# anzeA/Tarok

Measured on AMD Instinct MI355X. Metric: env steps/sec at 65 536 parallel 4-player games; 1/2/4/8 MI355X, higher is better.
Workload: dtype u64

## Files before the change

### tarok_amd/csrc/tarok_env.hip

```cpp
#include "tarok_device.h"

#include <hip/hip_runtime.h>
#include <stdint.h>
#include <stdio.h>
#include <stdlib.h>
#include <string.h>
#include <type_traits>
#include <utility>

#include "../../include/tarok_env.h"

#define TK_BLOCK 256
#define TK_PF_SLOTS (4 * TK_BLOCK)
#define TK_GRAPH_CACHE 16
#define TK_REFILL_CAP (TK_BLOCK * TK_AHEAD)
#define TK_REFILL_FAN 8
#define TK_RC(group, k) ((((size_t)(group)) * 4 + (k)) * 32)
#define TK_BULK_EVERY 32u
#define TK_BULK_CAP ((TK_BULK_EVERY / 4) * TK_BLOCK)

#define TK_AHEAD TAROK_GAMES_AHEAD
#define TK_LINE(episode) ((u32)(episode) % (u32)TK_AHEAD)
#define TK_FINQ 128
#define TK_STREAM_STORE(ptr, val) __builtin_nontemporal_store((val), (ptr))
#define TK_WAIT_LOADS() __builtin_amdgcn_s_waitcnt(0x0F70)
#define TK_RARE(c) __builtin_expect(!!(c), 0)
#define TK_USUAL(c) __builtin_expect(!!(c), 1)

struct __attribute__((aligned(64))) AuxLine {
    ulonglong2 n01, n23; u64 nkey; u32 nep;
    u32 pad[5];
};
struct __attribute__((aligned(64))) Aux { AuxLine line[TK_AHEAD]; };
static_assert(sizeof(AuxLine) == 64 && sizeof(Aux) == 64 * TK_AHEAD, "64 bytes per next-game line");
static_assert((TK_BLOCK * sizeof(Aux)) % 128 == 0, "a play group's next-game lines end on an L2 line boundary");
static_assert(TK_AHEAD >= 2 && TK_AHEAD <= 15, "epar / cprev are 4-bit fields");
struct __attribute__((aligned(32))) Counters {
    int4 score_sum;
    u32 episode;
    u32 pad[3];
};
static_assert(sizeof(Counters) == 32, "Counters is half a cache line");

struct tarok_env {
    int device;
    int64_t n;
    u64 offset, seed;
    int mix, flags;
    ulonglong2 *s01, *s23;
    Aux *aux;
    Counters *cnt;
    uint16_t *nstale;
    u64 *gkey;
    uint8_t *hist;
    u64 *rlist;
    u32 *rcount;
    u64 *elist;
    u32 *epoch;
    uint32_t refill_fan;
    uint32_t lazy_refill;
    int n_cus;
    float *adam_sumsq;
    u64 *stamps;
    size_t stamps_words;
    int launched;
    hipStream_t cap_stream;
    struct GraphEntry {
        hipGraphExec_t exec;
        int fused, chunk, flags, prefetch;
        void *action, *reward, *done, *obs, *stamps;
        uint32_t fan, lazy;
    } graphs[TK_GRAPH_CACHE];
    int n_graphs;
};

static thread_local int g_last_hip = 0;

#define HIPCHK(x)                                                   \
    do {                                                            \
        hipError_t e_ = (x);                                        \
        if (e_ != hipSuccess) { g_last_hip = (int)e_; return TAROK_EHIP; } \
    } while (0)

static inline dim3 grid_for(int64_t n) { return dim3((unsigned)((n + TK_BLOCK - 1) / TK_BLOCK)); }

// ... 270 lines not shown
            u32 base = 0;
#pragma unroll
            for (u32 r = 0; r < TK_REFILL_FAN; r++) base = (r == q) ? cum[r] : base;
            u64 en = tk_ld(&lists[((int64_t)(g0 + q) * 2 + which) * cap + (j - base)]);
            deal_into_buffer(aux, (int64_t)(g0 + q) * TK_BLOCK + (u32)(en & 0xFFFF), (u32)(en >> 32), seed, offset, mix);
        }
    }
    if (any || bulk) {
        __syncthreads();
        if (any && tid < fan && g0 + tid < play_groups) rcount[TK_RC(g0 + tid, par ^ 1u)] = 0u;
        if (bulk && tid < fan && g0 + tid < play_groups) rcount[TK_RC(g0 + tid, 2 + which)] = 0u;
    }
}

template <bool HIST>
__device__ __forceinline__ void play_role(
    u32 group, u32 tid,
    int64_t n, u64 seed, u64 offset, int mix, int flags, int cards, int64_t stride, TkCount count, u32 *epoch, u32 play_groups, u32 fan,
    uint8_t *__restrict__ action_out, int16_t *__restrict__ reward,
    uint8_t *__restrict__ done, uint16_t *__restrict__ trick, u64 *__restrict__ obs, uint8_t *__restrict__ hist,
    ulonglong2 *__restrict__ s01, ulonglong2 *__restrict__ s23, Aux *aux, Counters *__restrict__ cnt,
    u64 *__restrict__ gkey, u64 *rlist, u32 *rcount, u64 *__restrict__ stamps) {
    __shared__ unsigned short push_list[TK_REFILL_CAP];
    __shared__ u32 push_ep[TK_BLOCK];
    __shared__ u32 push_count;
    __shared__ u32 finq[TK_BLOCK / 64][9][TK_FINQ];
    __shared__ int sacc[4][TK_BLOCK];
    if (tid == 0) push_count = 0;
    sacc[0][tid] = 0; sacc[1][tid] = 0; sacc[2][tid] = 0; sacc[3][tid] = 0;
    __syncthreads();
    u32 fq_head = 0, fq_n = 0;
    u32 (*fq)[TK_FINQ] = finq[tid >> 6];
    auto drain_finished = [&](u32 cnt_) __attribute__((always_inline)) {
        u32 lane = tid & 63;
        if (lane < cnt_) {
            u32 e = (fq_head + lane) & (TK_FINQ - 1);
            Game f;
            f.A = TK_U64(fq[0][e], fq[1][e]); f.B = TK_U64(fq[2][e], fq[3][e]); f.C = TK_U64(fq[4][e], fq[5][e] & 0x3FFFFFu);
            u32 m = fq[7][e], ri = fq[8][e];
            f.talon = TK_U64(fq[6][e], (m >> 24) & 15u);
            f.contract = m & 15; f.declarer = (m >> 4) & 3; f.king = (m >> 6) & 3; f.team = (m >> 8) & 15;
            f.tl = (m >> 12) & 7; f.trick_no = (m >> 16) & 15; f.leader = (m >> 20) & 3;
            f.trick = 0; f.nt = 0; f.phase = TK_PHASE_DONE; f.error = 0; f.epar = 0; f.cprev = 0;
            u64 sc = final_scores(f);
            u32 t = ri & 0xFFFFu;
            if (reward) {
                u64 rs = sc;
                if ((flags & TAROK_REWARD_REF) && (f.contract == TK_BERAC || f.contract == TK_ODPRTI_BERAC)) {
                    int dv = f.trick_no >= 12 ? -20 : 20;
                    u32 d = f.declarer;
                    rs = pack_scores(d == 0 ? (int)(int16_t)(sc & 0xFFFF) : dv, d == 1 ? (int)(int16_t)((sc >> 16) & 0xFFFF) : dv,
                                     d == 2 ? (int)(int16_t)((sc >> 32) & 0xFFFF) : dv, d == 3 ? (int)(int16_t)(sc >> 48) : dv);
                }
                reinterpret_cast<u64 *>(reward)[(int64_t)group * TK_BLOCK + t + (int64_t)(ri >> 16) * stride] = rs;
            }
            atomicAdd(&sacc[0][t], (int)(int16_t)(sc & 0xFFFF)); atomicAdd(&sacc[1][t], (int)(int16_t)((sc >> 16) & 0xFFFF));
            atomicAdd(&sacc[2][t], (int)(int16_t)((sc >> 32) & 0xFFFF)); atomicAdd(&sacc[3][t], (int)(int16_t)(sc >> 48));
        }
        fq_head = (fq_head + cnt_) & (TK_FINQ - 1);
        fq_n -= cnt_;
    };
    u64 t_real0 = 0, t_cyc0 = 0, t_play = 0;
    if (stamps) { t_real0 = __builtin_amdgcn_s_memrealtime(); t_cyc0 = __builtin_amdgcn_s_memtime(); }
    int64_t i = (int64_t)group * TK_BLOCK + tid;
    bool valid = i < n;
    int64_t ic = valid ? i : n - 1;
    Game g;
    load_game(g, s01, s23, ic);
    u64 key = gkey[ic];
    bool autoreset = (flags & TAROK_AUTO_RESET) != 0;
    bool berac = g.contract == TK_BERAC || g.contract == TK_ODPRTI_BERAC;
    bool spec = valid && ((g.phase == TK_PHASE_PLAY && (int)g.nt + cards >= 4 &&
                           (berac || (int)(g.trick_no * 4 + g.nt) + cards >= 48)) ||
                          g.phase == TK_PHASE_DONE);
    u32 cprev0 = valid ? g.cprev : 0u;
    u32 allowed = TK_AHEAD - min(cprev0, (u32)TK_AHEAD);
    int4 acc = make_int4(0, 0, 0, 0);
    u32 cur_ep = 0;
    ulonglong2 na = make_ulonglong2(0, 0), nb = na, na2 = na, nb2 = na;
    u64 nkey = 0, nkey2 = 0;
    u32 nep1 = 0, nep2 = 0;
    bool ok1 = false, ok2 = false;
    auto line_tag = [&](bool &ok, u32 &nep, u32 tag) __attribute__((always_inline)) { nep = tag; ok = true; };
    if (spec) {
        acc = cnt[i].score_sum;
        cur_ep = cnt[i].episode;
        if (autoreset && allowed > 0) {
            const AuxLine *ln = &aux[i].line[TK_LINE(g.epar + 1)];
            na = ln->n01; nb = ln->n23; nkey = ln->nkey;
            line_tag(ok1, nep1, ln->nep);
            if (allowed > 1 && cards > 4) {
                const AuxLine *l2 = &aux[i].line[TK_LINE(g.epar + 2)];
                na2 = l2->n01; nb2 = l2->n23; nkey2 = l2->nkey;
                line_tag(ok2, nep2, l2->nep);
            }
        }
    }
    TK_WAIT_LOADS();
    u32 par = launch_phase<1>(count, play_groups, fan) & 1u;
    launch_counted<1>(epoch);
    g.cprev = 0;
    u32 consumed = 0;
    bool resync = false;
    bool blocked = false;
    bool acc_dirty = false, seats_dirty = false, touched = false;
    u64 legal = (valid && g.phase == TK_PHASE_PLAY) ? legal_now(g) : 0;
    u64 c_lead = 0;
    u32 legal_hi = 0;
    u64 pending = 0;
    u32 blocked_v = 0, resync_v = 0;
    auto fetch_lines = [&](bool lacks, bool lacks2) __attribute__((always_inline)) {
        if (lacks) {
            const AuxLine *ln = &aux[i].line[TK_LINE(cur_ep + 1)];
            na = ln->n01; nb = ln->n23; nkey = ln->nkey;
            line_tag(ok1, nep1, ln->nep);
        }
        if (lacks2) {
            const AuxLine *l2 = &aux[i].line[TK_LINE(cur_ep + 2)];
            na2 = l2->n01; nb2 = l2->n23; nkey2 = l2->nkey;
            line_tag(ok2, nep2, l2->nep);
        }
    };
    auto play_card = [&](auto all_tag, auto nt_tag, auto std_tag, int64_t row, int ci) __attribute__((always_inline)) {
        constexpr bool ALL = decltype(all_tag)::value;
        constexpr int NT = decltype(nt_tag)::value;
        constexpr bool STD = decltype(std_tag)::value;
        if constexpr (NT >= 0) g.nt = (u32)NT;
        constexpr bool TOP_UP_EARLY = ALL && NT == 0;
        constexpr bool TOP_UP_LATE = !(ALL && NT == 3);
        if constexpr (TOP_UP_EARLY) {
            if (TK_RARE(pending != 0)) {
                pending = 0;
                bool base = spec && blocked_v == 0 && consumed >= 1;
                bool lacks = base && nep1 != cur_ep + 1 && consumed < allowed;
                bool lacks2 = base && nep2 != cur_ep + 2 && consumed + 1 < allowed;
                fetch_lines(lacks, lacks2);
            }
        }
        const bool v = ALL ? true : valid;
        const bool play = ALL ? true : (valid && g.phase == TK_PHASE_PLAY);
        constexpr bool ALIGNED = ALL && NT >= 0;
        u32 a;
        if constexpr (ALL && NT >= 1) a = policy_action_follow(key, g.trick_no * 4 + g.nt, TK_LO(legal) | TK_HI(legal), legal_hi);
        else a = play ? policy_action(key, g.trick_no * 4 + g.nt, legal) : 255u;
        u64 scores = 0;
        u32 trick_info = 0;
        int res = -2;
        const u32 pos = g.trick_no * 4 + g.nt;
        if constexpr (ALL && NT == 0) c_lead = g.C;
        const u64 *lead_plane = (ALL && NT >= 0) ? &c_lead : nullptr;
        if (play) res = apply_step<true, true>(g, a, scores, trick_info, !STD && trick != nullptr, lead_plane);
        bool fin = res == 1;
        if (HIST && hist && play && res >= 0) hist[(int64_t)pos * n + i] = (uint8_t)a;
        if constexpr (!(ALL && NT >= 0)) {
            touched = touched || res != -2;
            seats_dirty = seats_dirty || (res >= 0 && g.nt == 0);
        }
        if (v) {
            if (STD || action_out) TK_STREAM_STORE(&action_out[row], (uint8_t)a);
            if (!STD && trick) TK_STREAM_STORE(&trick[row], (uint16_t)trick_info);
        }
        constexpr bool CAN_END = !(ALL && NT >= 0 && NT < 3);
        constexpr bool FAST_RENEW = ALL && NT == 3;
        auto push_finished = [&](u64 fm, u32 slot0) __attribute__((always_inline)) {
            u32 e = (slot0 + __builtin_amdgcn_mbcnt_hi((u32)(fm >> 32), __builtin_amdgcn_mbcnt_lo((u32)fm, 0))) & (TK_FINQ - 1);
            fq[0][e] = TK_LO(g.A); fq[1][e] = TK_HI(g.A); fq[2][e] = TK_LO(g.B); fq[3][e] = TK_HI(g.B);
            fq[4][e] = TK_LO(g.C); fq[5][e] = TK_HI(g.C); fq[6][e] = TK_LO(g.talon);
            u32 m = (g.declarer << 4) | g.contract;      TK_KEEP_VGPR(m);
            m = (g.king << 6) | m;                       TK_KEEP_VGPR(m);
            m = (g.team << 8) | m;                       TK_KEEP_VGPR(m);
            m = (g.tl << 12) | m;                        TK_KEEP_VGPR(m);
            m = (g.trick_no << 16) | m;                  TK_KEEP_VGPR(m);
            m = (g.leader << 20) | m;                    TK_KEEP_VGPR(m);
            fq[7][e] = (TK_HI(g.talon) << 24) | m;
            fq[8][e] = ((u32)ci << 16) | tid;
        };
        auto swap_in = [&]() __attribute__((always_inline)) {
            unpack_fresh(g, na.x, na.y, nb.x, nb.y);
            if constexpr (ALIGNED) g.C |= TK_C_PAD;
            key = nkey;
            na = na2; nb = nb2; nkey = nkey2;
            nep1 = nep2;
        };
        auto deal_in_place = [&](bool deal_here, Game &gd, u64 &kd) __attribute__((always_inline)) {
            u64 pend = __ballot(deal_here);
            if (TK_RARE(pend != 0)) {
                u64 dkey = 0;
                if (deal_here) dkey = game_key(seed, offset + (u64)i, cur_ep + 1);
                u64 h0 = 0, h1 = 0, h2 = 0, h3 = 0, tal = 0;
                u32 lane = __lane_id();
                while (pend) {
                    int l = __builtin_ctzll(pend);
                    pend &= pend - 1;
                    u32 klo = (u32)__builtin_amdgcn_readlane((int)(u32)dkey, l);
                    u32 khi = (u32)__builtin_amdgcn_readlane((int)(u32)(dkey >> 32), l);
                    u64 w0, w1, w2, w3, wt;
                    deal_wave(klo, khi, w0, w1, w2, w3, wt);
                    if (lane == (u32)l) { h0 = w0; h1 = w1; h2 = w2; h3 = w3; tal = wt; }
                }
                if (deal_here) {
                    u32 cc, d, k;
                    sample_setup(dkey, mix, cc, d, k);
                    setup_game(gd, h0, h1, h2, h3, tal, cc, d, k);
                    gd.epar = TK_LINE(cur_ep + 1); gd.cprev = 0;
                    if (gd.phase == TK_PHASE_EXCHANGE) bot_exchange(gd, dkey);
                    kd = dkey;
                }
            }
        };
        if constexpr (FAST_RENEW) {
            u64 fm = __ballot(fin);
            if (TK_USUAL(fm != 0)) {
                if (TK_RARE(fq_n >= 64)) drain_finished(64);
                const u32 slot0 = fq_head + fq_n;
                fq_n += (u32)__popcll(fm);
                if (TK_RARE((fm & __ballot(nep1 != cur_ep + 1)) != 0)) {
                    bool lineless = fin && nep1 != cur_ep + 1;
                    resync_v |= (lineless && consumed < allowed) ? 1u : 0u;
                    blocked_v |= lineless ? 1u : 0u;
                    Game d = g;
                    u64 dk = key;
                    deal_in_place(lineless, d, dk);
                    if (lineless) { pack(d, na.x, na.y, nb.x, nb.y); nkey = dk; nep1 = cur_ep + 1; }
                }
                pending |= fm & __ballot(nep2 != cur_ep + 2);
                if (fin) { push_finished(fm, slot0); swap_in(); cur_ep++; consumed++; }
            }
        }
        if constexpr (CAN_END && !FAST_RENEW) {
            u64 fm = __ballot(fin);
            if (TK_USUAL(fm != 0)) {
                if (TK_RARE(fq_n >= 64)) drain_finished(64);
                if (fin) push_finished(fm, fq_head + fq_n);
                fq_n += (u32)__popcll(fm);
            }
        }
        if (CAN_END && !FAST_RENEW && (ALL || autoreset)) {
            bool renew = ALL ? fin : (v && g.phase == TK_PHASE_DONE);
            if (TK_USUAL(__ballot(renew) != 0)) {
                if constexpr (TOP_UP_LATE) {
                    bool lacks = spec && !blocked && !ok1 && consumed >= 1 && consumed < allowed;
                    if (TK_RARE(__ballot(renew && lacks) != 0)) {
                        bool lacks2 = spec && !blocked && !ok2 && consumed >= 1 && consumed + 1 < allowed;
                        fetch_lines(lacks, lacks2);
                        TK_WAIT_LOADS();
                    }
                }
                bool swap = renew && !blocked && ok1 && nep1 == cur_ep + 1;
                if (swap) {
                    swap_in();
                    ok1 = ok2 && consumed + 1 < allowed;
                    ok2 = false;
                }
                bool deal_here = renew && !swap;
                if (deal_here && consumed < allowed) resync = true;
                if (deal_here) blocked = true;
                deal_in_place(deal_here, g, key);
                if (renew) { cur_ep++; consumed++; seats_dirty = true; }
            }
        }
        if constexpr (ALIGNED && NT < 3) legal = legal_mask_follow(hand_of<true>(g, (g.leader + g.nt) & 3), g.trick & 63, g.contract, legal_hi);
        else if constexpr (ALIGNED) legal = legal_mask(hand_of<true>(g, g.leader), false, 0u, g.contract);
        else legal = (ALL || (v && g.phase == TK_PHASE_PLAY)) ? legal_now(g) : 0;
        if (v) {
            const u32 fin01 = ALL ? (u32)res : (fin ? 1u : 0u);
            TK_STREAM_STORE(&obs[row], obs_word_with<true>(g, false, legal) | ((u64)(ALL ? fin01 : ((fin || g.phase == TK_PHASE_DONE) ? 1u : 0u)) << 62));
            if (STD || done) TK_STREAM_STORE(&done[row], (uint8_t)fin01);
        }
    };
    int64_t row = i;
    typedef std::integral_constant<int, -1> nt_any;
    if (autoreset && __ballot(valid && g.phase == TK_PHASE_PLAY) == ~0ULL) {
        if ((cards & 3) == 0 && __ballot(g.nt != 0) == 0) {
            auto tricks = [&](auto std_tag) __attribute__((always_inline)) {
                touched = true; seats_dirty = true;
                g.C |= TK_C_PAD;
                for (int c = 0; c < cards; c += 4) {
                    play_card(std::true_type{}, std::integral_constant<int, 0>{}, std_tag, row, c); row += stride;
                    play_card(std::true_type{}, std::integral_constant<int, 1>{}, std_tag, row, c + 1); row += stride;
                    play_card(std::true_type{}, std::integral_constant<int, 2>{}, std_tag, row, c + 2); row += stride;
                    play_card(std::true_type{}, std::integral_constant<int, 3>{}, std_tag, row, c + 3); row += stride;
                }
                g.C &= TK_DECK;
            };
            if (action_out && done && !trick) tricks(std::true_type{});
            else tricks(std::false_type{});
        } else {
            for (int c = 0; c < cards; c++, row += stride) play_card(std::true_type{}, nt_any{}, std::false_type{}, row, c);
        }
    } else {
        for (int c = 0; c < cards; c++, row += stride) play_card(std::false_type{}, nt_any{}, std::false_type{}, row, c);
    }
    while (fq_n) drain_finished(min(fq_n, 64u));
    __builtin_amdgcn_s_waitcnt(0xC07F);
    {
        int4 sa = make_int4(sacc[0][tid], sacc[1][tid], sacc[2][tid], sacc[3][tid]);
        if (sa.x | sa.y | sa.z | sa.w) { acc.x += sa.x; acc.y += sa.y; acc.z += sa.z; acc.w += sa.w; acc_dirty = true; }
    }
    u32 np = (resync || resync_v != 0) ? (u32)TK_AHEAD : min(consumed, (u32)TK_AHEAD);
    if (valid) {
        g.cprev = np;
        if (acc_dirty) cnt[i].score_sum = acc;
        if (consumed) { cnt[i].episode = cur_ep; gkey[i] = key; }
        if (touched || consumed || cprev0 != np) store_game(g, s01, s23, i, seats_dirty || cprev0 != np);
    }
    if (stamps) t_play = __builtin_amdgcn_s_memtime() - t_cyc0;
    if (valid && np) {
        u32 pos = atomicAdd(&push_count, np);
        push_ep[tid] = cur_ep;
        for (u32 j = 0; j < np; j++) push_list[pos + j] = (unsigned short)(j * TK_BLOCK + tid);
    }
    __syncthreads();
    u32 total = push_count;
    u64 *lst = rlist + ((int64_t)group * 2 + par) * TK_REFILL_CAP;
    for (u32 j = tid; j < total; j += TK_BLOCK) {
        u32 en = push_list[j], t = en % TK_BLOCK;
        lst[j] = ((u64)(push_ep[t] + TK_AHEAD - en / TK_BLOCK) << 32) | t;
    }
    if (tid == 0) rcount[TK_RC(group, par)] = total;
    if (stamps && (tid & 63) == 0) {
        u64 w = (u64)i >> 6;
        stamps[3 * w + 0] = t_real0;
        stamps[3 * w + 1] = __builtin_amdgcn_s_memrealtime();
        stamps[3 * w + 2] = ((__builtin_amdgcn_s_memtime() - t_cyc0) << 32) | (t_play & 0xFFFFFFFFULL);
    }
}

#define TK_PLAY_ARGS                                                                                                             \
    int64_t n, u64 seed, u64 offset, int mix, int flags, int cards, int64_t stride, u32 play_groups, u32 *epoch, u32 fan,         \
        uint8_t *__restrict__ action_out, int16_t *__restrict__ reward,                                                           \
        uint8_t *__restrict__ done, uint16_t *__restrict__ trick, u64 *__restrict__ obs, uint8_t *__restrict__ hist,              \
        ulonglong2 *__restrict__ s01, ulonglong2 *__restrict__ s23, Aux *aux, Counters *__restrict__ cnt,                         \
        u64 *__restrict__ gkey, u64 *rlist, u32 *rcount, u64 *__restrict__ stamps
template <bool HIST>
TK_KERNEL(TK_BLOCK, 168) __attribute__((amdgpu_waves_per_eu(3, 3))) void k_play_wide(TK_PLAY_ARGS) {
    TK_VGPR_TOP(168, 167);
    TkCount count = launch_count<1>(epoch, play_groups);
    if (blockIdx.x >= play_groups)
        refill_role<false>(blockIdx.x - play_groups, threadIdx.x, TK_BLOCK, seed, offset, mix, play_groups, count, epoch, fan, false, aux, rlist, rcount, nullptr);
    else {
        play_role<HIST>(blockIdx.x, threadIdx.x, n, seed, offset, mix, flags, cards, stride, count, epoch, play_groups, fan,
                        action_out, reward, done, trick, obs, hist, s01, s23, aux, cnt, gkey, rlist, rcount, stamps);
    }
}

__device__ __forceinline__ void deal_in_place_wave(bool deal_here, Game &gd, u64 &kd, u64 seed, u64 offset, int64_t i, u32 ep, int mix) {
    u64 pend = __ballot(deal_here);
    if (pend == 0) return;
    u64 dkey = 0;
    if (deal_here) dkey = game_key(seed, offset + (u64)i, ep);
    u64 h0 = 0, h1 = 0, h2 = 0, h3 = 0, tal = 0;
    u32 lane = __lane_id();
    while (pend) {
        int l = __builtin_ctzll(pend);
        pend &= pend - 1;
        u32 klo = (u32)__builtin_amdgcn_readlane((int)(u32)dkey, l);
// ... 1123 lines not shown
    TK_VGPR_TOP(64, 63);
    int64_t i = (int64_t)blockIdx.x * TK_BLOCK + threadIdx.x;
    if (i >= n) return;
    if (ep) ep[i] = cnt[i].episode;
    if (score_sum) score_sum[i] = cnt[i].score_sum;
}

TK_KERNEL(TK_BLOCK, 64) void k_get_state(int64_t n, const ulonglong2 *__restrict__ s01,
                                                       const ulonglong2 *__restrict__ s23, u64 *__restrict__ out) {
    TK_VGPR_TOP(64, 63);
    int64_t i = (int64_t)blockIdx.x * TK_BLOCK + threadIdx.x;
    if (i >= n) return;
    Game g;
    load_game(g, s01, s23, i);
    u64 on_table = 0;
    for (u32 j = 0; j < g.nt; j++) on_table |= 1ULL << ((g.trick >> (6 * j)) & 63);
    u64 won = g.C & ~talon_unowned(g) & ~on_table;
    for (u32 s = 0; s < 4; s++) {
        out[(int64_t)s * n + i] = hand_of(g, s);
        out[(int64_t)(4 + s) * n + i] = seat_cards(g, s) & won;
    }
    out[8 * n + i] = g.talon;
    u64 m = g.trick;
    m |= (u64)g.nt << 24;
    m |= (u64)g.leader << 27;
    m |= (u64)g.trick_no << 29;
    m |= (u64)g.contract << 33;
    m |= (u64)g.declarer << 37;
    m |= (u64)(has_king(g.contract) ? g.king : 7) << 39;
    m |= (u64)g.team << 42;
    m |= (u64)(g.contract == TK_KLOP ? g.tl : 0) << 46;
    m |= (u64)(has_exchange(g.contract) ? g.tl : 7) << 49;
    m |= (u64)g.phase << 52;
    m |= (u64)g.error << 54;
    out[9 * n + i] = m;
}

TK_KERNEL(TK_BLOCK, 64) void k_set_state(int64_t n, const u64 *__restrict__ in,
                                                       ulonglong2 *__restrict__ s01, ulonglong2 *__restrict__ s23,
                                                       const Counters *__restrict__ cnt) {
    TK_VGPR_TOP(64, 63);
    int64_t i = (int64_t)blockIdx.x * TK_BLOCK + threadIdx.x;
    if (i >= n) return;
    u64 m = in[9 * n + i];
    Game g;
    g.trick = (u32)m & 0xFFFFFF;
    g.nt = (u32)(m >> 24) & 7; g.leader = (u32)(m >> 27) & 3; g.trick_no = (u32)(m >> 29) & 15;
    g.contract = (u32)(m >> 33) & 15; g.declarer = (u32)(m >> 37) & 3;
    u32 king = (u32)(m >> 39) & 7;
    g.king = king == 7 ? 0 : king;
    g.team = (u32)(m >> 42) & 15;
    u32 talon_left = (u32)(m >> 46) & 7, choice = (u32)(m >> 49) & 7;
    g.phase = (u32)(m >> 52) & 3; g.error = (u32)(m >> 54) & 1;
    g.epar = TK_LINE(cnt[i].episode);
    {
        ulonglong2 old = s23[i];
        g.cprev = ((u32)(old.y >> 62) & 3u) | (((u32)(old.x >> 62) & 3u) << 2);
    }
    g.talon = in[8 * n + i] & ((1ULL << 36) - 1);
    g.tl = g.contract == TK_KLOP ? talon_left : ((has_exchange(g.contract) || g.contract == TK_SOLO_BREZ) ? choice : 0);
    u64 seatc[4];
    u64 piles = 0;
    for (u32 s = 0; s < 4; s++) {
        u64 h = in[(int64_t)s * n + i] & TK_DECK, p = in[(int64_t)(4 + s) * n + i] & TK_DECK;
        seatc[s] = h | p;
        piles |= p;
    }
    u64 on_table = 0;
    for (u32 j = 0; j < g.nt && j < 4; j++) {
        u64 b = 1ULL << ((g.trick >> (6 * j)) & 63);
        on_table |= b;
        seatc[(g.leader + j) & 3] |= b;
    }
    u64 unowned = talon_unowned(g);
    u32 o = g.contract == TK_KLOP ? 0u : (u32)__builtin_ctz(~g.team & 15u);
    seatc[o & 3] |= unowned;
    g.A = seatc[1] | seatc[3];
    g.B = seatc[2] | seatc[3];
    g.C = piles | on_table | unowned;
    store_game(g, s01, s23, i);
}


__global__ __launch_bounds__(TK_BLOCK) TK_VGPR_BUDGET(64) void k_dbg_fill_lists(u64 *rlist, u32 *rcount, u32 per_slot, u32 ep0, u32 order) {
    TK_VGPR_TOP(64, 63);
    u32 g = blockIdx.x;
    for (u32 idx = threadIdx.x; idx < per_slot * TK_BLOCK; idx += TK_BLOCK) {
        u32 k = idx / TK_BLOCK, t = idx % TK_BLOCK;
        if (order == 1) t = TK_BLOCK - 1 - t;
        if (order == 2) t = (t * 37u + 11u) % TK_BLOCK;
        u64 en = ((u64)(ep0 + 1 + k) << 32) | t;
        rlist[((int64_t)g * 2 + 0) * TK_REFILL_CAP + idx] = en;
        rlist[((int64_t)g * 2 + 1) * TK_REFILL_CAP + idx] = en;
    }
    if (threadIdx.x == 0) {
        rcount[TK_RC(g, 0)] = per_slot * TK_BLOCK; rcount[TK_RC(g, 1)] = per_slot * TK_BLOCK;
        rcount[TK_RC(g, 2)] = 0; rcount[TK_RC(g, 3)] = 0;
    }
}
__global__ __launch_bounds__(TK_BLOCK) TK_VGPR_BUDGET(64) void k_dbg_clear_lines(Aux *aux, int64_t n) {
    TK_VGPR_TOP(64, 63);
    int64_t i = (int64_t)blockIdx.x * TK_BLOCK + threadIdx.x;
    if (i >= n) return;
    for (int b = 0; b < TK_AHEAD; b++) {
        AuxLine *ln = &aux[i].line[b];
        ln->n01 = make_ulonglong2(0, 0); ln->n23 = make_ulonglong2(0, 0); ln->nkey = 0; ln->nep = 0xFFFFFFFFu;
    }
}
__global__ __launch_bounds__(TK_BLOCK) TK_VGPR_BUDGET(128) void k_dbg_check_lines(Aux *aux, int64_t n, u64 seed, u64 offset, int mix, u32 per_slot,
                                                                                  u32 ep0, unsigned long long *out) {
    TK_VGPR_TOP(128, 127);
    int64_t i = (int64_t)blockIdx.x * TK_BLOCK + threadIdx.x;
    if (i >= n) return;
    for (u32 k = 0; k < per_slot; k++) {
        u32 episode = ep0 + 1 + k;
        u64 key = game_key(seed, offset + (u64)i, (u64)episode);
        u64 h0, h1, h2, h3, tal;
        deal_thread(key, h0, h1, h2, h3, tal);
        u32 c, d, kk;
        sample_setup(key, mix, c, d, kk);
        Game g;
        setup_game(g, h0, h1, h2, h3, tal, c, d, kk);
        g.epar = TK_LINE(episode); g.cprev = 0;
        if (g.phase == TK_PHASE_EXCHANGE) bot_exchange(g, key);
        ulonglong2 ea, eb;
        pack(g, ea.x, ea.y, eb.x, eb.y);
        const AuxLine *ln = &aux[i].line[TK_LINE(episode)];
        ulonglong2 na = ln->n01, nb = ln->n23;
        if (ea.x != na.x || ea.y != na.y || eb.x != nb.x || eb.y != nb.y || key != ln->nkey || ln->nep != episode) {
            unsigned long long r = atomicAdd(&out[0], 1ULL);
            if (r < 8) {
                unsigned long long *o = out + 1 + 6 * r;
                o[0] = (u64)i; o[1] = episode; o[2] = na.x; o[3] = ea.x; o[4] = nb.x; o[5] = eb.x;
            }
        }
    }
}

extern "C" {

const char *tarok_strerror(int code) {
    switch (code) {
        case TAROK_OK: return "ok";
        case TAROK_EINVAL: return "invalid argument";
        case TAROK_EHIP: return "HIP runtime error (see tarok_last_hip_error)";
        case TAROK_ENOMEM: return "out of device memory";
        case TAROK_ENODEV: return "no usable GPU";
        default: return "unknown error";
    }
}

int tarok_abi_version(void) { return TAROK_ABI_VERSION; }
int tarok_last_hip_error(void) { return g_last_hip; }

int tarok_device_count(void) {
    int n = 0;
    if (hipGetDeviceCount(&n) != hipSuccess) { (void)hipGetLastError(); return 0; }
    return n;
}

int tarok_create(tarok_env **out, int device, int64_t n_games, uint64_t game_offset, uint64_t seed, int mix, int flags) {
    if (!out || n_games <= 0 || n_games > (1LL << 31) || (flags & ~TAROK_HISTORY)) return TAROK_EINVAL;
    if (!(mix == TAROK_MIX_ALL || mix == TAROK_MIX_NAVADNA3 || mix == TAROK_MIX_BOT || (mix >= TAROK_MIX_FIXED && mix < TAROK_MIX_FIXED + 10))) return TAROK_EINVAL;
    if (device < 0 || device >= tarok_device_count()) return TAROK_ENODEV;
    HIPCHK(hipSetDevice(device));
    tarok_env *e = new tarok_env();
    memset(e, 0, sizeof *e);
    e->device = device; e->n = n_games; e->offset = game_offset; e->seed = seed; e->mix = mix; e->flags = flags;
    e->refill_fan = n_games >= (1 << 20) ? TK_REFILL_FAN : (n_games >= (1 << 18) ? 4 : 1);
    e->lazy_refill = n_games < (1 << 20) ? 1 : 0;
    size_t stale_bytes = (size_t)((n_games + TK_PF_SLOTS - 1) / TK_PF_SLOTS) * TK_PF_SLOTS * sizeof(uint16_t);
    hipError_t r = hipMalloc((void **)&e->s01, (size_t)n_games * sizeof(ulonglong2));
    if (r == hipSuccess) r = hipMalloc((void **)&e->s23, (size_t)n_games * sizeof(ulonglong2));
    if (r == hipSuccess) r = hipMalloc((void **)&e->aux, (size_t)n_games * sizeof(Aux));
    if (r == hipSuccess) r = hipMalloc((void **)&e->cnt, (size_t)n_games * sizeof(Counters));
    if (r == hipSuccess) r = hipMalloc((void **)&e->nstale, stale_bytes);
    if (r == hipSuccess) r = hipMalloc((void **)&e->gkey, (size_t)n_games * sizeof(u64));
    if (r == hipSuccess && (flags & TAROK_HISTORY)) r = hipMalloc((void **)&e->hist, (size_t)n_games * 48);
    if (r == hipSuccess && e->hist) r = hipMemset(e->hist, 255, (size_t)n_games * 48);
// ... 193 lines not shown
    if (prefetch_every % unit != 0) return TAROK_EINVAL;
    if (graph_chunk > 0 && prefetch_every > 0 && graph_chunk % prefetch_every != 0) return TAROK_EINVAL;
    if (!(flags & TAROK_AUTO_RESET)) prefetch_every = 0;
    if (cards_per_launch == 0 && !action) return TAROK_EINVAL;
    HIPCHK(hipSetDevice(e->device));
    hipStream_t s = (hipStream_t)stream;
    int64_t left = n_steps;
    if (graph_chunk > 0 && left >= graph_chunk) {
        hipGraphExec_t gexec = nullptr;
        for (int k = 0; k < e->n_graphs && !gexec; k++) {
            const tarok_env::GraphEntry &g = e->graphs[k];
            if (g.fused == cards_per_launch && g.chunk == graph_chunk && g.flags == flags && g.prefetch == prefetch_every &&
                g.action == action && g.reward == reward_out && g.done == done_out && g.obs == obs_out && g.stamps == e->stamps &&
                g.fan == e->refill_fan && g.lazy == e->lazy_refill)
                gexec = g.exec;
        }
        if (!gexec) {
            if (e->n_graphs == TK_GRAPH_CACHE) drop_graphs(e);
            hipGraph_t graph = nullptr;
            HIPCHK(hipStreamBeginCapture(e->cap_stream, hipStreamCaptureModeRelaxed));
            for (int k = 0; k < graph_chunk; k += unit) {
                launch_one(e, cards_per_launch, action, reward_out, done_out, obs_out, flags, e->cap_stream);
                if (prefetch_every && (k + unit) % prefetch_every == 0) launch_prefetch(e, e->cap_stream);
            }
            HIPCHK(hipStreamEndCapture(e->cap_stream, &graph));
            hipError_t r = hipGraphInstantiate(&gexec, graph, nullptr, nullptr, 0);
            (void)hipGraphDestroy(graph);
            if (r != hipSuccess) { g_last_hip = (int)r; return TAROK_EHIP; }
            e->graphs[e->n_graphs++] = {gexec, cards_per_launch, graph_chunk, flags, prefetch_every, action, reward_out, done_out,
                                        obs_out, e->stamps, e->refill_fan, e->lazy_refill};
        }
        while (left >= graph_chunk) {
            HIPCHK(hipGraphLaunch(gexec, s));
            left -= graph_chunk;
        }
    }
    for (int64_t k = 0; left > 0; left -= unit, k += unit) {
        launch_one(e, cards_per_launch, action, reward_out, done_out, obs_out, flags, s);
        if (prefetch_every && (k + unit) % prefetch_every == 0) launch_prefetch(e, s);
    }
    HIPCHK(hipGetLastError());
    return TAROK_OK;
}

int tarok_rollout_random(tarok_env *e, uint32_t episode, int16_t *scores_out, int16_t *nsteps_out, int8_t *seats_out,
                         uint64_t *masks_out, uint8_t *actions_out, void *stream) {
    if (!e) return TAROK_EINVAL;
    HIPCHK(hipSetDevice(e->device));
    hipLaunchKernelGGL(k_rollout, grid_for(e->n), dim3(TK_BLOCK), 0, (hipStream_t)stream, e->n, e->seed, e->offset,
                       episode, e->mix, scores_out, nsteps_out, seats_out, (u64 *)masks_out, actions_out);
    HIPCHK(hipGetLastError());
    return TAROK_OK;
}

int tarok_debug_stamps_sized(tarok_env *e, uint64_t *stamps, int64_t n_words) {
    if (!e || n_words < 0 || (stamps && n_words == 0)) return TAROK_EINVAL;
    e->stamps = (u64 *)stamps;
    e->stamps_words = stamps ? (size_t)n_words : 0;
    return TAROK_OK;
}

int tarok_debug_stamps(tarok_env *e, uint64_t *stamps) {
    if (!e) return TAROK_EINVAL;
    return tarok_debug_stamps_sized(e, stamps, stamps ? 3 * ((e->n + 63) / 64) : 0);
}

int tarok_debug_refill_selftest(tarok_env *e, int kind, int per_slot, uint32_t episode0, int order, int reps, uint64_t *report_out) {
    if (!e || kind < 0 || kind > 3 || per_slot < 1 || per_slot > TK_AHEAD || order < 0 || order > 2 || reps < 1 || !report_out) return TAROK_EINVAL;
    HIPCHK(hipSetDevice(e->device));
    const int64_t n = e->n;
    const size_t rows = 4;
    void *buf = nullptr;
    unsigned long long *rep = nullptr;
    HIPCHK(hipMalloc(&buf, rows * (size_t)n * (8 + 8 + 1 + 1) + 64));
    hipError_t r = hipMalloc((void **)&rep, 49 * sizeof(unsigned long long));
    if (r == hipSuccess) r = hipMemset(rep, 0, 49 * sizeof(unsigned long long));
    if (r != hipSuccess) { (void)hipFree(buf); g_last_hip = (int)r; return TAROK_EHIP; }
    uint64_t *obs = (uint64_t *)buf;
    int16_t *reward = (int16_t *)(obs + rows * n);
    uint8_t *action = (uint8_t *)(reward + rows * n * 4), *done = action + rows * n;
    u32 groups = (u32)((n + TK_BLOCK - 1) / TK_BLOCK);
    for (int it = 0; it < reps; it++) {
        hipLaunchKernelGGL(k_dbg_clear_lines, grid_for(n), dim3(TK_BLOCK), 0, 0, e->aux, n);
        hipLaunchKernelGGL(k_dbg_fill_lists, dim3(groups), dim3(TK_BLOCK), 0, 0, e->rlist, e->rcount, (u32)per_slot, episode0, (u32)order);
        if (kind == 0) launch_play(e, true, 1, n, nullptr, action, reward, done, nullptr, obs, TAROK_AUTO_RESET, 0);
        else if (kind == 1) {
            hipLaunchKernelGGL(k_legal, grid_for(n), dim3(TK_BLOCK), 0, 0, n, e->s01, e->s23, (u64 *)obs, (int8_t *)nullptr);
            launch_policy(e, obs, action, 0);
            launch_play(e, false, 1, n, action, nullptr, reward, done, nullptr, obs, TAROK_AUTO_RESET, 0);
        } else launch_play(e, true, kind == 2 ? 4 : 2, n, nullptr, action, reward, done, nullptr, obs, TAROK_AUTO_RESET, 0);
        hipLaunchKernelGGL(k_dbg_check_lines, grid_for(n), dim3(TK_BLOCK), 0, 0, e->aux, n, e->seed, e->offset, e->mix, (u32)per_slot, episode0, rep);
    }
    r = hipDeviceSynchronize();
    if (r == hipSuccess) r = hipMemcpy(report_out, rep, 49 * sizeof(unsigned long long), hipMemcpyDeviceToHost);
    if (r == hipSuccess) r = hipMemset(e->rcount, 0, TK_RC(groups, 0) * sizeof(u32));
    if (r == hipSuccess) {
        hipLaunchKernelGGL(k_dbg_clear_lines, grid_for(n), dim3(TK_BLOCK), 0, 0, e->aux, n);
        r = hipDeviceSynchronize();
    }
    (void)hipFree(buf); (void)hipFree(rep);
    if (r != hipSuccess) { g_last_hip = (int)r; return TAROK_EHIP; }
    return TAROK_OK;
}

int tarok_observe(tarok_env *e, void *features_out, void *stream) {
    if (!e || !features_out) return TAROK_EINVAL;
    HIPCHK(hipSetDevice(e->device));
    hipLaunchKernelGGL(k_observe, grid_for(e->n), dim3(TK_BLOCK), 0, (hipStream_t)stream, e->n, e->s01, e->s23,
                       (uint2 *)features_out);
    HIPCHK(hipGetLastError());
    return TAROK_OK;
}

int tarok_observe_ref(tarok_env *e, uint8_t *record_out, int32_t *meta_out, void *stream) {
    if (!e || !record_out) return TAROK_EINVAL;
    if (!e->hist) return TAROK_EINVAL;
    HIPCHK(hipSetDevice(e->device));
    hipLaunchKernelGGL(k_observe_ref, dim3((unsigned)((e->n + OR_GAMES - 1) / OR_GAMES)), dim3(256), 0, (hipStream_t)stream, e->n,
                       e->s01, e->s23, e->hist, (uint4 *)record_out, (int4 *)meta_out);
    HIPCHK(hipGetLastError());
    return TAROK_OK;
}

int tarok_observe_exchange_ref(tarok_env *e, uint8_t *out, void *stream) {
    if (!e || !out) return TAROK_EINVAL;
    HIPCHK(hipSetDevice(e->device));
    hipLaunchKernelGGL(k_observe_exchange_ref, grid_for(e->n), dim3(TK_BLOCK), 0, (hipStream_t)stream, e->n, e->s01, e->s23,
                       (uint2 *)out);
    HIPCHK(hipGetLastError());
    return TAROK_OK;
}

int tarok_observe_hands_ref(tarok_env *e, uint8_t *out, void *stream) {
    if (!e || !out) return TAROK_EINVAL;
    HIPCHK(hipSetDevice(e->device));
    hipLaunchKernelGGL(k_observe_hands_ref, grid_for(e->n), dim3(TK_BLOCK), 0, (hipStream_t)stream, e->n, e->s01, e->s23,
                       (uint2 *)out);
    HIPCHK(hipGetLastError());
    return TAROK_OK;
}

int tarok_get_history(tarok_env *e, uint8_t *hist_out, void *stream) {
    if (!e || !hist_out || !e->hist) return TAROK_EINVAL;
    HIPCHK(hipSetDevice(e->device));
    HIPCHK(hipMemcpyAsync(hist_out, e->hist, (size_t)e->n * 48, hipMemcpyDeviceToDevice, (hipStream_t)stream));
    return TAROK_OK;
}

int tarok_set_history(tarok_env *e, const uint8_t *hist_in, void *stream) {
    if (!e || !hist_in || !e->hist) return TAROK_EINVAL;
    HIPCHK(hipSetDevice(e->device));
    HIPCHK(hipMemcpyAsync(e->hist, hist_in, (size_t)e->n * 48, hipMemcpyDeviceToDevice, (hipStream_t)stream));
    return TAROK_OK;
}

int tarok_sample_policy(tarok_env *e, const void *logits_bf16, const uint64_t *obs, uint8_t *action_out,
                        float *logp_out, void *stream) {
    if (!e || !logits_bf16 || !obs || !action_out) return TAROK_EINVAL;
    HIPCHK(hipSetDevice(e->device));
    hipLaunchKernelGGL(k_sample, grid_for(e->n), dim3(TK_BLOCK), 0, (hipStream_t)stream, e->n, (const uint4 *)logits_bf16,
                       (const u64 *)obs, e->gkey, action_out, logp_out);
    HIPCHK(hipGetLastError());
    return TAROK_OK;
}

int tarok_policy_mlp(tarok_env *e, const void *w1, const float *b1, const void *w2, const float *b2, const void *w3,
                     const float *b3, const uint64_t *obs, uint8_t *action_out, float *logp_out, float *value_out,
// ... 278 lines not shown
```

Baseline: 190.0 billion.

## Drop second look-ahead line prefetch in aligned fast path; merge key/tag load

In the aligned all-play path, the kernel no longer preloads the second look-ahead aux line. Instead it re-fetches the next line at the start of each trick when the current one is stale, replacing the pending/blocked bookkeeping with a single limit counter. Each line's key and tag are now read as one 12-byte vector load. The intent is to cut registers and memory traffic in the hot loop, at the cost of possibly exposing load latency on the per-trick refetch. The debug refill list filler also now handles partial last blocks.

```diff
diff --git a/tarok_amd/csrc/tarok_env.hip b/tarok_amd/csrc/tarok_env.hip
--- a/tarok_amd/csrc/tarok_env.hip
+++ b/tarok_amd/csrc/tarok_env.hip
@@ -1,6 +1,7 @@
 #include "tarok_device.h"
 
 #include <hip/hip_runtime.h>
+#include <stddef.h>
 #include <stdint.h>
 #include <stdio.h>
 #include <stdlib.h>
@@ -437,18 +438,22 @@
     u32 nep1 = 0, nep2 = 0;
     bool ok1 = false, ok2 = false;
     auto line_tag = [&](bool &ok, u32 &nep, u32 tag) __attribute__((always_inline)) { nep = tag; ok = true; };
+    static_assert(offsetof(AuxLine, nkey) == 32 && offsetof(AuxLine, nep) == 40, "key and tag share the line's third 16 bytes");
+    auto load_line = [&](const AuxLine *ln, ulonglong2 &a, ulonglong2 &b, u64 &k, bool &ok, u32 &nep) __attribute__((always_inline)) {
+        a = ln->n01; b = ln->n23;
+        uint3 kt = *reinterpret_cast<const uint3 *>(__builtin_assume_aligned(&ln->nkey, 16));
+        k = TK_U64(kt.x, kt.y);
+        line_tag(ok, nep, kt.z);
+    };
+    const bool all_play = autoreset && __ballot(valid && g.phase == TK_PHASE_PLAY) == ~0ULL;
+    const bool aligned = all_play && (cards & 3) == 0 && __ballot(g.nt != 0) == 0;
     if (spec) {
         acc = cnt[i].score_sum;
         cur_ep = cnt[i].episode;
         if (autoreset && allowed > 0) {
-            const AuxLine *ln = &aux[i].line[TK_LINE(g.epar + 1)];
-            na = ln->n01; nb = ln->n23; nkey = ln->nkey;
-            line_tag(ok1, nep1, ln->nep);
-            if (allowed > 1 && cards > 4) {
-                const AuxLine *l2 = &aux[i].line[TK_LINE(g.epar + 2)];
-                na2 = l2->n01; nb2 = l2->n23; nkey2 = l2->nkey;
-                line_tag(ok2, nep2, l2->nep);
-            }
+            load_line(&aux[i].line[TK_LINE(g.epar + 1)], na, nb, nkey, ok1, nep1);
+            if (!aligned && allowed > 1 && cards > 4)
+                load_line(&aux[i].line[TK_LINE(g.epar + 2)], na2, nb2, nkey2, ok2, nep2);
         }
     }
     TK_WAIT_LOADS();
@@ -462,19 +467,11 @@
     u64 legal = (valid && g.phase == TK_PHASE_PLAY) ? legal_now(g) : 0;
     u64 c_lead = 0;
     u32 legal_hi = 0;
-    u64 pending = 0;
-    u32 blocked_v = 0, resync_v = 0;
+    u32 resync_v = 0;
+    u32 lim = spec ? allowed : 0u;
     auto fetch_lines = [&](bool lacks, bool lacks2) __attribute__((always_inline)) {
-        if (lacks) {
-            const AuxLine *ln = &aux[i].line[TK_LINE(cur_ep + 1)];
-            na = ln->n01; nb = ln->n23; nkey = ln->nkey;
-            line_tag(ok1, nep1, ln->nep);
-        }
-        if (lacks2) {
-            const AuxLine *l2 = &aux[i].line[TK_LINE(cur_ep + 2)];
-            na2 = l2->n01; nb2 = l2->n23; nkey2 = l2->nkey;
-            line_tag(ok2, nep2, l2->nep);
-        }
+        if (lacks) load_line(&aux[i].line[TK_LINE(cur_ep + 1)], na, nb, nkey, ok1, nep1);
+        if (lacks2) load_line(&aux[i].line[TK_LINE(cur_ep + 2)], na2, nb2, nkey2, ok2, nep2);
     };
     auto play_card = [&](auto all_tag, auto nt_tag, auto std_tag, int64_t row, int ci) __attribute__((always_inline)) {
         constexpr bool ALL = decltype(all_tag)::value;
@@ -484,12 +481,9 @@
         constexpr bool TOP_UP_EARLY = ALL && NT == 0;
         constexpr bool TOP_UP_LATE = !(ALL && NT == 3);
         if constexpr (TOP_UP_EARLY) {
-            if (TK_RARE(pending != 0)) {
-                pending = 0;
-                bool base = spec && blocked_v == 0 && consumed >= 1;
-                bool lacks = base && nep1 != cur_ep + 1 && consumed < allowed;
-                bool lacks2 = base && nep2 != cur_ep + 2 && consumed + 1 < allowed;
-                fetch_lines(lacks, lacks2);
+            if (nep1 != cur_ep + 1 && consumed < lim) {
+                u32 off = g.epar + 1 >= (u32)TK_AHEAD ? 0u : (g.epar + 1) * (u32)sizeof(AuxLine);
+                load_line(reinterpret_cast<const AuxLine *>(reinterpret_cast<const char *>(aux[i].line) + off), na, nb, nkey, ok1, nep1);
             }
         }
         const bool v = ALL ? true : valid;
@@ -534,8 +528,10 @@
             unpack_fresh(g, na.x, na.y, nb.x, nb.y);
             if constexpr (ALIGNED) g.C |= TK_C_PAD;
             key = nkey;
-            na = na2; nb = nb2; nkey = nkey2;
-            nep1 = nep2;
+            if constexpr (!ALIGNED) {
+                na = na2; nb = nb2; nkey = nkey2;
+                nep1 = nep2;
+            }
         };
         auto deal_in_place = [&](bool deal_here, Game &gd, u64 &kd) __attribute__((always_inline)) {
             u64 pend = __ballot(deal_here);
@@ -565,20 +561,20 @@
         };
         if constexpr (FAST_RENEW) {
             u64 fm = __ballot(fin);
+            const u64 nol = __ballot(nep1 != cur_ep + 1);
             if (TK_USUAL(fm != 0)) {
                 if (TK_RARE(fq_n >= 64)) drain_finished(64);
                 const u32 slot0 = fq_head + fq_n;
                 fq_n += (u32)__popcll(fm);
-                if (TK_RARE((fm & __ballot(nep1 != cur_ep + 1)) != 0)) {
+                if (TK_RARE((fm & nol) != 0)) {
                     bool lineless = fin && nep1 != cur_ep + 1;
-                    resync_v |= (lineless && consumed < allowed) ? 1u : 0u;
-                    blocked_v |= lineless ? 1u : 0u;
+                    resync_v |= (lineless && consumed < lim) ? 1u : 0u;
+                    lim = lineless ? 0u : lim;
                     Game d = g;
                     u64 dk = key;
                     deal_in_place(lineless, d, dk);
                     if (lineless) { pack(d, na.x, na.y, nb.x, nb.y); nkey = dk; nep1 = cur_ep + 1; }
                 }
-                pending |= fm & __ballot(nep2 != cur_ep + 2);
                 if (fin) { push_finished(fm, slot0); swap_in(); cur_ep++; consumed++; }
             }
         }
@@ -625,8 +621,8 @@
     };
     int64_t row = i;
     typedef std::integral_constant<int, -1> nt_any;
-    if (autoreset && __ballot(valid && g.phase == TK_PHASE_PLAY) == ~0ULL) {
-        if ((cards & 3) == 0 && __ballot(g.nt != 0) == 0) {
+    if (all_play) {
+        if (aligned) {
             auto tricks = [&](auto std_tag) __attribute__((always_inline)) {
                 touched = true; seats_dirty = true;
                 g.C |= TK_C_PAD;
@@ -1916,19 +1912,21 @@
 }
 
 
-__global__ __launch_bounds__(TK_BLOCK) TK_VGPR_BUDGET(64) void k_dbg_fill_lists(u64 *rlist, u32 *rcount, u32 per_slot, u32 ep0, u32 order) {
+__global__ __launch_bounds__(TK_BLOCK) TK_VGPR_BUDGET(64) void k_dbg_fill_lists(u64 *rlist, u32 *rcount, int64_t n, u32 per_slot, u32 ep0, u32 order) {
     TK_VGPR_TOP(64, 63);
     u32 g = blockIdx.x;
-    for (u32 idx = threadIdx.x; idx < per_slot * TK_BLOCK; idx += TK_BLOCK) {
-        u32 k = idx / TK_BLOCK, t = idx % TK_BLOCK;
-        if (order == 1) t = TK_BLOCK - 1 - t;
-        if (order == 2) t = (t * 37u + 11u) % TK_BLOCK;
+    const u32 have = (u32)min((int64_t)TK_BLOCK, n - (int64_t)g * TK_BLOCK);
+    if (order == 2 && have % 37u == 0) order = 1;
+    for (u32 idx = threadIdx.x; idx < per_slot * have; idx += TK_BLOCK) {
+        u32 k = idx / have, t = idx % have;
+        if (order == 1) t = have - 1 - t;
+        if (order == 2) t = (t * 37u + 11u) % have;
         u64 en = ((u64)(ep0 + 1 + k) << 32) | t;
         rlist[((int64_t)g * 2 + 0) * TK_REFILL_CAP + idx] = en;
         rlist[((int64_t)g * 2 + 1) * TK_REFILL_CAP + idx] = en;
     }
     if (threadIdx.x == 0) {
-        rcount[TK_RC(g, 0)] = per_slot * TK_BLOCK; rcount[TK_RC(g, 1)] = per_slot * TK_BLOCK;
+        rcount[TK_RC(g, 0)] = per_slot * have; rcount[TK_RC(g, 1)] = per_slot * have;
         rcount[TK_RC(g, 2)] = 0; rcount[TK_RC(g, 3)] = 0;
     }
 }
@@ -2288,7 +2286,7 @@
     u32 groups = (u32)((n + TK_BLOCK - 1) / TK_BLOCK);
     for (int it = 0; it < reps; it++) {
         hipLaunchKernelGGL(k_dbg_clear_lines, grid_for(n), dim3(TK_BLOCK), 0, 0, e->aux, n);
-        hipLaunchKernelGGL(k_dbg_fill_lists, dim3(groups), dim3(TK_BLOCK), 0, 0, e->rlist, e->rcount, (u32)per_slot, episode0, (u32)order);
+        hipLaunchKernelGGL(k_dbg_fill_lists, dim3(groups), dim3(TK_BLOCK), 0, 0, e->rlist, e->rcount, n, (u32)per_slot, episode0, (u32)order);
         if (kind == 0) launch_play(e, true, 1, n, nullptr, action, reward, done, nullptr, obs, TAROK_AUTO_RESET, 0);
         else if (kind == 1) {
             hipLaunchKernelGGL(k_legal, grid_for(n), dim3(TK_BLOCK), 0, 0, n, e->s01, e->s23, (u64 *)obs, (int8_t *)nullptr);
```

Measured after the change: 193.3 billion, median of 6. +1.7%, better.
